# Ego-J/I2VSGG

Measured on AMD Instinct MI355X. Metric: frames/sec (600x1000, 32 ROI/frame), higher is better.
Workload: dtype f32; 1 GPU; BASELINE.json configs[1]: cfgs/res101.yml, SGG_emb fwd+bwd+SGD, 2 frames/GPU 600x1000, 32 boxes + 32 pairs/frame, ResNet-101 C4; frames_per_gpu=2, global_frames=2, hip_graph=True, parallelism=dp1 (frames sharded, RCCL all-reduce of vrd grads)

## Files before the change

### i2vsgg_amd/_lib.py

```python
import ctypes as C
import os

import torch

_HERE = os.path.dirname(os.path.abspath(__file__))
LIB_PATH = os.path.join(_HERE, "libi2vsgg_hip.so")

LAYOUT_NHWC, LAYOUT_NCHW = 0, 1
EPI_RELU, EPI_RESIDUAL, EPI_SCALE, EPI_BIAS, EPI_ZEROED = 1, 2, 4, 8, 16

_p, _i, _f, _z, _l = C.c_void_p, C.c_int32, C.c_float, C.c_size_t, C.c_int64

SIGNATURES = {
    "i2v_version": (_i, []),
    "i2v_last_error": (C.c_char_p, []),
    "i2v_build_flags": (_i, []),
    "i2v_stream_create": (_i, [_i, _i, C.POINTER(C.c_void_p)]),
    "i2v_stream_destroy": (_i, [_p]),
    "i2v_roi_align_fwd": (_i, [_p, _i, _i, _i, _i, _i, _p, _i, _i, _i, _f, _i, _p, _i, _p]),
    "i2v_roi_align_bwd": (_i, [_p, _i, _p, _i, _i, _i, _f, _i, _p, _i, _i, _i, _i, _i, _p]),
    "i2v_roi_align_bwd_gather_workspace_bytes": (_z, [_i, _i, _i, _i, _i]),
    "i2v_roi_align_bwd_gather": (_i, [_p, _p, _i, _i, _i, _f, _i, _p, _i, _i, _i, _i, _p, _z, _p]),
    "i2v_roi_align_sampled_fwd": (_i, [_p, _i, _i, _i, _i, _i, _p, _i, _i, _i, _f, _i, _p, _i, _p]),
    "i2v_roi_align_sampled_bwd": (_i, [_p, _i, _p, _i, _i, _i, _f, _i, _p, _i, _i, _i, _i, _i, _p]),
# ... 20 lines not shown
    "i2v_winograd4_filter": (_i, [_p, _p, _i, _i, _p]),
    "i2v_winograd4_filter_dgrad": (_i, [_p, _p, _i, _i, _p]),
    "i2v_conv3x3_winograd4_workspace_bytes": (_z, [_i, _i, _i, _i, _i]),
    "i2v_conv3x3_winograd4_fwd": (_i, [_p, _p, _p, _p, _p, _i, _i, _i, _i, _i, _i, _p, _z, _p]),
    "i2v_conv_set_tile": (_i, [_i]),
    "i2v_conv_debug_clock": (_i, [_p]),
    "i2v_debug_clock_stamp": (_i, [_p, _p]),
    "i2v_conv_dgrad_workspace_bytes": (_z, [_i, _i, _i, _i]),
    "i2v_conv_dgrad": (_i, [_p, _p, _p, _i, _i, _i, _i, _i, _i, _i, _i, _i, _p, _z, _p, _z, _p]),
    "i2v_conv_wgrad_workspace_bytes": (_z, [_i, _i, _i, _i, _i, _i, _i, _i, _i]),
    "i2v_conv_wgrad": (_i, [_p, _p, _p, _i, _i, _i, _i, _i, _i, _i, _i, _i, _f, _p, _z, _p]),
    "i2v_conv_dgrad_fused": (_i, [_p, _p, _p, _p, _p, _p, _p, _i, _i, _i, _i, _i, _i, _i, _i, _i, _p, _z, _p, _z, _p]),
    "i2v_conv_wgrad_scaled": (_i, [_p, _p, _p, _p, _i, _i, _i, _i, _i, _i, _i, _i, _i, _f, _p, _z, _p]),
    "i2v_ordered_fallbacks": (_i, [_i]),
    "i2v_conv3x3_winograd4_dgrad": (_i, [_p, _p, _p, _p, _p, _i, _i, _i, _i, _i, _p, _z, _p]),
    "i2v_conv3x3_winograd4_wgrad_workspace_bytes": (_z, [_i, _i, _i, _i, _i]),
    "i2v_conv3x3_winograd4_wgrad": (_i, [_p, _p, _p, _p, _i, _i, _i, _i, _i, _f, _p, _z, _p]),
    "i2v_gemm_tn_batched": (_i, [_p, _p, _p, _i, _i, _i, _i, _l, _l, _l, _p]),
    "i2v_gemm_tn_batched_acc": (_i, [_p, _p, _p, _i, _i, _i, _i, _l, _l, _l, _p]),
    "i2v_conv3x3_winograd4_v_bytes": (_z, [_i, _i, _i, _i]),
    "i2v_conv3x3_winograd4_fwd_keep": (_i, [_p, _p, _p, _p, _p, _p, _i, _i, _i, _i, _i, _i, _p, _z, _p]),
    "i2v_conv3x3_winograd4_wgrad_v": (_i, [_p, _p, _p, _p, _i, _i, _i, _i, _i, _f, _p, _z, _p]),
    "i2v_conv_wgrad_sgd": (_i, [_p, _p, _p, _p, _i, _i, _i, _i, _i, _i, _i, _i, _i, _f, _f, _f, _p]),
    "i2v_epilogue_bwd": (_i, [_p, _p, _p, _p, _p, _p, _l, _i, _i, _p, _p, _z, _p]),
    "i2v_maxpool3x3s2_fwd": (_i, [_p, _p, _p, _i, _i, _i, _i, _p]),
    "i2v_sgd_momentum": (_i, [_p, _p, _p, _l, _f, _f, _f, _p]),
    "i2v_sgd_momentum_multi": (_i, [_p, _p, _p, _p, _p, _p, _i, _f, _p]),
    "i2v_adam_step": (_i, [_p, _p]),
    "i2v_adam_multi": (_i, [_p, _p, _p, _p, _p, _p, _p, _i, C.c_double, C.c_double, C.c_double, _p, _p]),
    "i2v_dstyle_pool_fwd": (_i, [_p, _p, _p, _l, _i, _i, _i, _p]),
    "i2v_dstyle_pool_bwd": (_i, [_p, _p, _p, _p, _p, _l, _i, _i, _i, _p]),
    "i2v_dstyle_fused_workspace_bytes": (_z, [_l, _i, _i, _i]),
    "i2v_dstyle_fused_fwd": (_i, [_p, _p, _p, _p, _p, _p, _p, _p, _l, _i, _i, _i, _i, _p, _z, _p]),
    "i2v_relation_topk_workspace_bytes": (_z, [_i, _i]),
    "i2v_relation_topk": (_i, [_p, _p, _p, _p, _i, _i, _i, _p, _p, _p, _p, _z, _p]),
    "i2v_image_prep_size": (_i, [_i, _i, _i, _p, _p, _p]),
    "i2v_image_prep": (_i, [_p, _i, _i, _i, _i, _p, _i, _p, _i, _i, _p]),
    "i2v_det_postprocess_workspace_bytes": (_z, [_i, _i]),
    "i2v_det_postprocess": (_i, [_p, _p, _p, _i, _p, _p, _f, _f, _f, _i, _i, _f, _f, _i, _p, _p, _p, _z, _p]),
    "i2v_det_postprocess_info": (_i, [_p, _p, _p, _i, _p, _p, _p, _i, _i, _f, _f, _i, _p, _p, _p, _z, _p]),
    "i2v_l2norm_rows_fwd": (_i, [_p, _p, _p, _i, _i, _f, _p]),
    "i2v_l2norm_rows_bwd": (_i, [_p, _p, _p, _p, _i, _i, _f, _p]),
    "i2v_bce_rows_fwd": (_i, [_p, _p, _p, _p, _i, _i, _p]),
    "i2v_bce_rows_bwd": (_i, [_p, _p, _p, _p, _p, _i, _i, _p]),
    "i2v_half_mse_fwd": (_i, [_p, _l, _f, _p, _p]),
    "i2v_half_mse_bwd": (_i, [_p, _l, _f, _p, _p, _p]),
    "i2v_smooth_l1_fwd": (_i, [_p, _p, _p, _p, _l, _i, _i, _f, _p, _p]),
    "i2v_smooth_l1_bwd": (_i, [_p, _p, _p, _p, _l, _i, _i, _f, _p, _p, _p]),
    "i2v_bbox_transform": (_i, [_p, _i, _p, _i, _p, _i, _i, _p, _p, _p]),
    "i2v_signed_sqrt_fwd": (_i, [_p, _p, _l, _p]),
    "i2v_signed_sqrt_bwd": (_i, [_p, _p, _p, _l, _p]),
    "i2v_pair_gather_fwd": (_i, [_p, _p, _p, _p, _i, _i, _i, _p]),
    "i2v_pair_gather_bwd": (_i, [_p, _p, _p, _p, _i, _i, _i, _p]),
    "i2v_dpixel_fwd": (_i, [_p, _p, _p, _p, _p, _p, _p, _p, _i, _i, _p]),
    "i2v_dpixel_bwd_workspace_bytes": (_z, []),
    "i2v_dpixel_bwd": (_i, [_p, _p, _p, _p, _p, _p, _p, _p, _p, _p, _p, _p, _i, _i, _f, _p, _z, _p]),
}


class I2VError(RuntimeError):
    pass


def _load():
    if not os.path.exists(LIB_PATH):
        raise ImportError(
            "i2vsgg_amd: %s not found. Build it with `python -c 'import __graft_entry__ as g; g.build()'` "
            "(hipcc --offload-arch=gfx950). There is no CPU fallback." % LIB_PATH)
    lib = C.CDLL(LIB_PATH)
    for name, (res, args) in SIGNATURES.items():
        try:
            fn = getattr(lib, name)
        except AttributeError:
            raise ImportError("i2vsgg_amd: %s does not export %s (stale build?)" % (LIB_PATH, name))
        fn.restype, fn.argtypes = res, args
    return lib


lib = _load()

TUNE = {"I2V_CONV_SPEC": 0, "I2V_SPLIT_TARGET": 1, "I2V_SPLIT_TARGET_SKINNY": 2, "I2V_SPLIT_BELOW": 3, "I2V_SPLIT_ATOMICS": 4,
        "I2V_BIG_FC_TILE": 5, "I2V_WGRAD_V2": 6, "I2V_WGRAD_FUSED_TILE": 7, "I2V_WINO_ROWS": 8, "I2V_ROIPOOL_C128": 9, "I2V_CONV_GEMM": 10, "I2V_STAGGER": 11, "I2V_ROIALIGN_COLS": 12, "I2V_WGRAD_PER_CU": 13, "I2V_WGRAD_XCD": 14, "I2V_FC_FOLD": 15, "I2V_GEMM_X3": 16,
        "I2V_GEMM_PERSIST": 17, "I2V_WGRAD_PRIO": 18, "I2V_STREAM_TILE": 19, "I2V_KGROUPS": 20, "I2V_WGRAD_ORDERED_GFLOP": 21, "I2V_GEMM_DMA": 22,
        "I2V_WGRAD_DMA": 23, "I2V_ROIALIGN_BWD": 24, "I2V_NMS_SCAN": 25}
ENV_TUNE = ("I2V_SPLIT_ATOMICS", "I2V_SPLIT_TARGET", "I2V_SPLIT_TARGET_SKINNY", "I2V_SPLIT_BELOW", "I2V_BIG_FC_TILE",
            "I2V_WGRAD_FUSED_TILE", "I2V_WGRAD_PER_CU", "I2V_KGROUPS", "I2V_WGRAD_ORDERED_GFLOP", "I2V_WINO_ROWS", "I2V_GEMM_DMA", "I2V_WGRAD_DMA", "I2V_ROIALIGN_BWD", "I2V_NMS_SCAN")
RETIRED_ENV = ("I2V_WINOGRAD_TRAIN", "I2V_BLOCK_FUSED", "I2V_WINOGRAD_WGRAD", "I2V_KEEP_V", "I2V_WGRAD_BRANCH", "I2V_ISD_BATCHED",
               "I2V_DEFER_FC", "I2V_EXPERIMENTS")
for _name, _key in TUNE.items():
    if os.environ.get(_name) in (None, ""):
        continue
    if _name not in ENV_TUNE:
        raise ImportError("i2vsgg_amd: %s is set but is not an environment knob (README.md lists them); it would be ignored. "
                          "Use i2vsgg_amd._lib.lib.i2v_set_tuning(TUNE[%r], value) from a tool or test" % (_name, _name))
    if lib.i2v_set_tuning(_key, int(os.environ[_name])) != 0:
        raise ImportError("i2vsgg_amd: %s=%s refused: %s" % (_name, os.environ[_name], lib.i2v_last_error().decode()))
for _name in RETIRED_ENV:
    if os.environ.get(_name) not in (None, ""):
        import warnings
        warnings.warn("i2vsgg_amd: %s is set but no longer read (a settled switch of rounds 1-5): the default runs" % _name)


def check(rc, what):
    if rc != 0:
        raise I2VError("%s failed (%d): %s" % (what, rc, lib.i2v_last_error().decode()))


def ptr(t):
    return None if t is None else t.data_ptr()


def stream():
    import torch
    return torch.cuda.current_stream().cuda_stream
```

### i2vsgg_amd/csrc/api.cpp

```cpp
#include <hip/hip_runtime.h>
#include <stdarg.h>
#include <stdio.h>
#include "../../include/i2vsgg_hip.h"

static thread_local char g_err[512] = "";

void i2v_set_error(const char* fmt, ...) {
    va_list ap;
    va_start(ap, fmt);
    vsnprintf(g_err, sizeof(g_err), fmt, ap);
    va_end(ap);
}

extern "C" int32_t i2v_version(void) { return 100; }
extern "C" const char* i2v_last_error(void) { return g_err; }

int g_i2v_tuning[I2V_TUNE_COUNT] = {
     -1,  2,  -1,  256,  2,
     1,  1,  128,  0,  1,
     1,  0,  2,  4,  1,
     0,  0,  0,  0,  1,
     0,  1000000,  1,  1,  1,  2,
};

extern "C" int32_t i2v_build_flags(void) {
    return 0;
}

extern "C" int32_t i2v_set_tuning(int32_t key, int32_t value) {
    if (key < 0 || key >= I2V_TUNE_COUNT) {
        i2v_set_error("set_tuning: unknown key %d", key);
        return I2V_ERR_ARG;
    }
    const bool retired = key == I2V_TUNE_CONV_SPEC ? value > 0
                       : (key == I2V_TUNE_FC_FOLD || key == I2V_TUNE_GEMM_X3 || key == I2V_TUNE_GEMM_PERSIST ||
                          key == I2V_TUNE_WGRAD_PRIO || key == I2V_TUNE_STAGGER) ? value != 0 : false;
    if (retired) {
        i2v_set_error("set_tuning: key %d belonged to an experiment kernel that is no longer in the library", key);
        return I2V_ERR_UNSUPPORTED;
    }
    g_i2v_tuning[key] = value;
    return I2V_OK;
}


extern "C" int32_t i2v_get_tuning(int32_t key) {
    return (key < 0 || key >= I2V_TUNE_COUNT) ? I2V_ERR_ARG : g_i2v_tuning[key];
}

extern "C" int32_t i2v_stream_create(int32_t device, int32_t priority, void** stream) {
    if (!stream) {
        i2v_set_error("stream_create: null output");
        return I2V_ERR_ARG;
    }
    int prev = -1, n = 0;
    if (hipGetDeviceCount(&n) != hipSuccess || device < 0 || device >= n) {
        i2v_set_error("stream_create: no device %d (%d visible)", device, n);
        return I2V_ERR_ARG;
    }
    hipStream_t s = nullptr;
    hipError_t e = hipGetDevice(&prev);
    if (e == hipSuccess && prev != device) e = hipSetDevice(device);
    if (e == hipSuccess) {
        int lo = 0, hi = 0;
        e = hipDeviceGetStreamPriorityRange(&lo, &hi);
        if (e == hipSuccess) {
            int pr = priority < hi ? hi : (priority > lo ? lo : priority);
            e = hipStreamCreateWithPriority(&s, hipStreamNonBlocking, pr);
        }
    }
    if (prev >= 0 && prev != device) (void)hipSetDevice(prev);
    if (e != hipSuccess) {
        i2v_set_error("stream_create: %s", hipGetErrorString(e));
        return I2V_ERR_LAUNCH;
    }
    *stream = (void*)s;
    return I2V_OK;
}

extern "C" int32_t i2v_stream_destroy(void* stream) {
    if (!stream) return I2V_OK;
    hipError_t e = hipStreamDestroy((hipStream_t)stream);
    if (e != hipSuccess) {
        i2v_set_error("stream_destroy: %s", hipGetErrorString(e));
        return I2V_ERR_LAUNCH;
    }
    return I2V_OK;
}
```

### i2vsgg_amd/csrc/conv.hip

```cpp
#include "common.h"
#include <algorithm>
#include <type_traits>
#include <stdlib.h>

namespace {

typedef float f32x16 __attribute__((ext_vector_type(16)));
typedef float f32x4 __attribute__((ext_vector_type(4)));
typedef unsigned int u32x4 __attribute__((ext_vector_type(4)));
typedef __bf16 bf16x4 __attribute__((ext_vector_type(4)));
typedef __bf16 bf16x8 __attribute__((ext_vector_type(8)));

constexpr int BK = 16;
constexpr int KTAB_MAX = 2560;
constexpr int BKS = 32;
constexpr int LDS_ROW = 20;
constexpr int THREADS = 256;
constexpr int kSplitInKernelMax = 4;

struct ConvP {
    const float* x; const float* w; const float* scale; const float* shift; const float* res; float* y;
    const float* mask;
    int B, H, W, Cin, Cout, KH, KW, stride, pad, Ho, Wo;
    int pad_x;
// ... 1926 lines not shown
            if (gpre) *(float4*)(gpre + r * N + n) = v;
            if (g) *(float4*)(g + r * N + n) = make_float4(v.x * sc.x, v.y * sc.y, v.z * sc.z, v.w * sc.w);
        }
    }
    if (!gbias) return;
    *(float4*)&red[threadIdx.x * 4] = s;
    __syncthreads();
    float4 t = make_float4(0.f, 0.f, 0.f, 0.f);
    if (threadIdx.x < cg) {
        for (int l = 0; l < lanes; ++l) {
            const float4 u = *(const float4*)&red[(l * cg + threadIdx.x) * 4];
            t.x += u.x; t.y += u.y; t.z += u.z; t.w += u.w;
        }
    }
    colsum_finish4(t, (int)(threadIdx.x % cg) * 4, N, threadIdx.x < cg, gbias, part, cnt);
}

__global__ void __launch_bounds__(256)
epilogue_bwd_scalar_kernel(const float* __restrict__ gy, const float* __restrict__ y, const float* __restrict__ scale,
                           float* __restrict__ g, float* __restrict__ gpre, float* __restrict__ gbias, long long M,
                           int N, int relu, int rows_per_blk, float* __restrict__ g_t, float* __restrict__ part) {
    const int n = blockIdx.y * 256 + threadIdx.x;
    if (n >= N) return;
    const long long r0 = (long long)blockIdx.x * rows_per_blk;
    const long long r1 = r0 + rows_per_blk < M ? r0 + rows_per_blk : M;
    const float sc = scale ? scale[n] : 1.f;
    float s = 0.f;
    for (long long r = r0; r < r1; ++r) {
        float v = gy[r * N + n];
        if (relu && !(y[r * N + n] > 0.f)) v = 0.f;
        s += v;
        if (gpre) gpre[r * N + n] = v;
        if (g) g[r * N + n] = v * sc;
        if (g_t) g_t[(long long)n * M + r] = v * sc;
    }
    if (gbias && part) part[(long long)blockIdx.x * N + n] = s;
    else if (gbias) atomicAdd(gbias + n, s);
}

}


extern "C" int32_t i2v_ordered_fallbacks(int32_t reset) {
    const int n = g_ordered_fallbacks;
    if (reset) g_ordered_fallbacks = 0;
    return n;
}

namespace {
__global__ void __launch_bounds__(256)
wgrad_reduce_kernel(const float* __restrict__ part, float* __restrict__ gw, int splits, int planes, long long nk4, long long bsw, int acc) {
    const long long total = (long long)planes * nk4;
    for (long long e = blockIdx.x * 256ll + threadIdx.x; e < total; e += 256ll * gridDim.x) {
        const long long plane = e / nk4, i = e - plane * nk4;
        float4* o = (float4*)(gw + plane * bsw) + i;
        float4 v = acc ? *o : make_float4(0.f, 0.f, 0.f, 0.f);
        const float4* src = (const float4*)part + plane * nk4 + i;
        for (int s0 = 0; s0 < splits; s0 += 8) {
            float4 u[8];
#pragma unroll
            for (int k = 0; k < 8; ++k) u[k] = s0 + k < splits ? src[(long long)(s0 + k) * planes * nk4] : make_float4(0.f, 0.f, 0.f, 0.f);
#pragma unroll
            for (int k = 0; k < 8; ++k)
                if (s0 + k < splits) { v.x += u[k].x; v.y += u[k].y; v.z += u[k].z; v.w += u[k].w; }
        }
        *o = v;
    }
}
__global__ void __launch_bounds__(256)
wgrad_reduce_scalar_kernel(const float* __restrict__ part, float* __restrict__ gw, int splits, long long nk, int acc) {
    for (long long e = blockIdx.x * 256ll + threadIdx.x; e < nk; e += 256ll * gridDim.x) {
        float v = acc ? gw[e] : 0.f;
        for (int s0 = 0; s0 < splits; s0 += 16) {
            float u[16];
#pragma unroll
            for (int k = 0; k < 16; ++k) u[k] = s0 + k < splits ? part[(long long)(s0 + k) * nk + e] : 0.f;
#pragma unroll
            for (int k = 0; k < 16; ++k)
                if (s0 + k < splits) v += u[k];
        }
        gw[e] = v;
    }
}
}

constexpr int kWgradOrderedMax = 16;

static int wgrad_split_count(long long M, int N, int K, int planes, int tm, int tk, int rs) {
    const long long tiles = (long long)i2v_cdiv(N, tm) * i2v_cdiv(K, tk), all_tiles = tiles * planes;
    const int msteps = i2v_cdiv(M, rs), per_cu = g_i2v_tuning[I2V_TUNE_WGRAD_PER_CU];
    int splits = (int)((long long)per_cu * NUM_CU / all_tiles);
    if (splits < 2) splits = (int)(((long long)per_cu * NUM_CU + all_tiles - 1) / all_tiles);
    if (splits > msteps / 4) splits = msteps / 4;
    if (splits < 1) splits = 1;
    return splits;
}

int i2v_internal_wgrad_plane_splits(long long T, int Cout, int Cin) {
    const int s = wgrad_split_count(T, Cout, Cin, 36, 64, 64, BKS);
    const int mps = i2v_cdiv(i2v_cdiv(T, BKS), s) * BKS;
    return i2v_cdiv(T, mps);
}

static bool launch_wgrad(WgP& p, float beta, bool fused, hipStream_t st, void* split_ws = nullptr, size_t split_ws_bytes = 0) {
    const long long xb = (long long)p.B * p.H * p.W * p.Cin * 4, gb = (long long)p.M * p.N * 4;
    const bool v2 = (p.N % 4 == 0) && xb < (1ll << 31) && gb < (1ll << 31) && g_wgrad_v2;
    if (p.row_scale && !v2) { i2v_set_error("conv_wgrad_scaled: shape outside the v2 kernel (Cout % 4, 2 GiB operands)"); return false; }
    int tm = 64, tk = 64;
    if (v2 && fused && g_wgrad_fused_tile == 128 && p.N >= 128) tm = 128;
    if (v2 && g_wgrad_v2 >= 2) {
        if (p.N >= 128) tm = 128;
        if (p.K >= 128 && tm == 128 && g_wgrad_v2 == 2) tk = 128;
    }
    const long long tiles = (long long)i2v_cdiv(p.N, tm) * i2v_cdiv(p.K, tk);
    const int rs = v2 ? BKS : 16;
    int splits = 1;
    const int msteps = i2v_cdiv(p.M, rs);
    if (!fused) splits = wgrad_split_count(p.M, p.N, p.K, p.nbatch > 1 ? p.nbatch : 1, tm, tk, rs);
    const int planes = p.nbatch > 1 ? p.nbatch : 1;
    const bool ext_part = p.part_ws != nullptr;
    const double ord_flops = 1e9 * g_i2v_tuning[I2V_TUNE_WGRAD_ORDERED_GFLOP], flops = 2.0 * p.M * p.N * p.K * planes;
    const bool want_ord = !fused && !ext_part && splits > 1 && g_i2v_tuning[I2V_TUNE_SPLIT_ATOMICS] == 0 && flops < ord_flops;
    if (want_ord && split_ws && v2 && splits > kWgradOrderedMax && flops < 1e9) splits = kWgradOrderedMax;
    if (ext_part && splits > p.part_cap) splits = p.part_cap > 0 ? p.part_cap : 1;
    p.m_per_split = i2v_cdiv(msteps, splits) * rs;
    splits = i2v_cdiv(p.M, p.m_per_split);
    p.direct = (splits == 1 && beta == 0.f) || fused;
    bool two_pass = false;
    if (ext_part) {
        if (splits == 1) p.part_ws = nullptr;
    } else if (want_ord && splits > 1) {
        const size_t need_ord = kSplitCounterBytes + (size_t)splits * tiles * planes * (size_t)(tm * tk) * sizeof(float);
        const size_t need_part = kSplitCounterBytes + (size_t)splits * planes * (size_t)p.N * p.K * sizeof(float);
        if (split_ws && v2 && splits <= kWgradOrderedMax && tiles * planes <= kSplitCounters && need_ord <= split_ws_bytes && need_ord < (1ull << 31)) {
            p.ord_cnt = reinterpret_cast<int*>(split_ws);
            p.ord_ws = reinterpret_cast<float*>(static_cast<char*>(split_ws) + kSplitCounterBytes);
            p.ord_splits = splits; p.ord_tiles = (int)tiles; p.ord_acc = beta != 0.f;
        } else if (split_ws && need_part <= split_ws_bytes) {
            p.part_ws = reinterpret_cast<float*>(static_cast<char*>(split_ws) + kSplitCounterBytes);
            two_pass = true;
        } else {
            ++g_ordered_fallbacks;
        }
    }
    if (beta == 0.f && !p.direct && !p.ord_ws && !p.part_ws)
        hipMemsetAsync(p.gw, 0, (p.nbatch > 1 ? (size_t)(p.nbatch - 1) * p.bsw : 0) * sizeof(float) + (size_t)p.N * p.K * sizeof(float), st);
    p.x_bytes = (unsigned)xb;
    p.gy_bytes = (unsigned)gb;
    dim3 grid((unsigned)tiles, splits, p.nbatch > 1 ? p.nbatch : 1);
    const long long groups = (long long)splits * (p.nbatch > 1 ? p.nbatch : 1), total = tiles * groups;
    p.xcd_remap = (v2 && groups >= 2 && total < (1ll << 30) && g_i2v_tuning[I2V_TUNE_WGRAD_XCD]) ? 1 : 0;
    if (p.xcd_remap) {
        p.r_tiles = (int)tiles; p.r_splits = splits; p.r_total = (int)total;
        grid = dim3((unsigned)((total + 7) / 8 * 8), 1, 1);
    }
    const bool lin = p.KH == 1 && p.KW == 1 && p.pad == 0 && p.stride == 1;
    const bool dma = v2 && !fused && !g_clk && lin && (p.K % 4 == 0) && g_i2v_tuning[I2V_TUNE_WGRAD_DMA];
    if (!v2) conv_wgrad_f32<64, 64><<<grid, THREADS, 0, st>>>(p);
    else if (dma && tm == 128 && tk == 128) conv_wgrad2_f32<4, 4, false, false, true><<<grid, THREADS, 0, st>>>(p);
    else if (dma && tm == 128) conv_wgrad2_f32<4, 2, false, false, true><<<grid, THREADS, 0, st>>>(p);
    else if (dma) conv_wgrad2_f32<2, 2, false, false, true><<<grid, THREADS, 0, st>>>(p);
    else if (fused && tm == 128 && tk == 64) conv_wgrad2_f32<4, 2, true><<<grid, THREADS, 0, st>>>(p);
    else if (tm == 128 && tk == 128) conv_wgrad2_f32<4, 4><<<grid, THREADS, 0, st>>>(p);
    else if (tm == 128) conv_wgrad2_f32<4, 2><<<grid, THREADS, 0, st>>>(p);
    else if (fused) conv_wgrad2_f32<2, 2, true><<<grid, THREADS, 0, st>>>(p);
    else if (g_clk) { p.clk = g_clk; p.abl = g_ablate; conv_wgrad2_f32<2, 2, false, true><<<grid, THREADS, 0, st>>>(p); }
// ... 239 lines not shown
    return I2V_OK;
}

static int32_t gemm_tn_batched_impl(const float* x, const float* gy, float* gw, int32_t M, int32_t N, int32_t K, int32_t nbatch,
                                    long long stride_x, long long stride_gy, long long stride_gw, float beta, void* stream,
                                    int part_cap = 0, int* part_splits = nullptr) {
    I2V_CHECK_ARG(x && gy && gw && M > 0 && N > 0 && K > 0 && nbatch > 0, "gemm_tn_batched: bad argument");
    I2V_CHECK_ARG(N % 4 == 0 && K % 4 == 0, "gemm_tn_batched: N and K must be multiples of 4");
    I2V_CHECK_ARG(nbatch == 1 || stride_gw == (long long)N * K, "gemm_tn_batched: gw batches must be contiguous");
    WgP p = {};
    p.x = x; p.gy = gy; p.gw = gw;
    p.B = 1; p.H = 1; p.W = M; p.Cin = K; p.Cout = N; p.KH = 1; p.KW = 1; p.stride = 1; p.pad = 0;
    p.Ho = 1; p.Wo = M;
    p.M = M; p.N = N; p.K = K;
    p.lgCin = ilog2_exact(K);
    p.nbatch = nbatch; p.bsx = stride_x; p.bsg = stride_gy; p.bsw = stride_gw;
    if (!g_wgrad_v2 || (long long)M * K * 4 >= (1ll << 31) || (long long)M * N * 4 >= (1ll << 31)) {
        i2v_set_error("gemm_tn_batched: operand larger than 2 GiB per batch");
        return I2V_ERR_UNSUPPORTED;
    }
    if (part_splits) {
        p.part_ws = gw; p.part_cap = part_cap;
    }
    launch_wgrad(p, beta, false, (hipStream_t)stream);
    if (part_splits) *part_splits = p.part_ws ? p.ord_splits : 1;
    I2V_CHECK_LAUNCH("gemm_tn_batched");
    return I2V_OK;
}

int32_t i2v_internal_reduce_parts(float* parts, int nparts, int planes, long long nk, void* stream) {
    const long long total = (long long)planes * (nk / 4);
    wgrad_reduce_kernel<<<(unsigned)std::min<long long>(i2v_cdiv(total, 256), 4096), 256, 0, (hipStream_t)stream>>>(
        parts, parts, nparts, planes, nk / 4, nk, 0);
    return I2V_OK;
}

int32_t i2v_internal_gemm_tn_batched_parts(const float* x, const float* gy, float* parts, int32_t M, int32_t N, int32_t K,
                                           int32_t nbatch, long long stride_x, long long stride_gy, int cap, int* splits, void* stream) {
    return gemm_tn_batched_impl(x, gy, parts, M, N, K, nbatch, stride_x, stride_gy, (long long)N * K, 0.f, stream, cap, splits);
}

extern "C" int32_t i2v_gemm_tn_batched(const float* x, const float* gy, float* gw, int32_t M, int32_t N, int32_t K,
                                       int32_t nbatch, long long stride_x, long long stride_gy, long long stride_gw,
                                       void* stream) {
    return gemm_tn_batched_impl(x, gy, gw, M, N, K, nbatch, stride_x, stride_gy, stride_gw, 0.f, stream);
}

extern "C" int32_t i2v_gemm_tn_batched_acc(const float* x, const float* gy, float* gw, int32_t M, int32_t N, int32_t K,
                                           int32_t nbatch, long long stride_x, long long stride_gy, long long stride_gw,
                                           void* stream) {
    return gemm_tn_batched_impl(x, gy, gw, M, N, K, nbatch, stride_x, stride_gy, stride_gw, 1.f, stream);
}

extern "C" int32_t i2v_conv_wgrad(const float* x, const float* gy, float* gw, int32_t B, int32_t H, int32_t W,
                                  int32_t Cin, int32_t Cout, int32_t KH, int32_t KW, int32_t stride, int32_t pad,
                                  float beta, void* ws, size_t ws_bytes, void* stream) {
    return conv_wgrad_impl(x, gy, gw, nullptr, B, H, W, Cin, Cout, KH, KW, stride, pad, beta, stream, ws, ws_bytes);
}

extern "C" int32_t i2v_conv_wgrad_scaled(const float* x, const float* gy, const float* row_scale, float* gw, int32_t B,
                                         int32_t H, int32_t W, int32_t Cin, int32_t Cout, int32_t KH, int32_t KW,
                                         int32_t stride, int32_t pad, float beta, void* ws, size_t ws_bytes, void* stream) {
    return conv_wgrad_impl(x, gy, gw, row_scale, B, H, W, Cin, Cout, KH, KW, stride, pad, beta, stream, ws, ws_bytes);
}

extern "C" int32_t i2v_conv_wgrad_sgd(const float* x, const float* gy, float* w, float* m, int32_t B, int32_t H,
                                      int32_t W, int32_t Cin, int32_t Cout, int32_t KH, int32_t KW, int32_t stride,
                                      int32_t pad, float lr, float momentum, float weight_decay, void* stream) {
    int rc = check_conv("conv_wgrad_sgd", x, gy, w, B, H, W, Cin, Cout, KH, KW, stride, pad);
    if (rc) return rc;
    I2V_CHECK_ARG(m, "conv_wgrad_sgd: null momentum buffer");
    WgP p = {};
    p.x = x; p.gy = gy; p.gw = w; p.sgd_m = m; p.lr = lr; p.mom = momentum; p.wd = weight_decay;
    p.B = B; p.H = H; p.W = W; p.Cin = Cin; p.Cout = Cout; p.KH = KH; p.KW = KW; p.stride = stride; p.pad = pad;
    p.Ho = (H + 2 * pad - KH) / stride + 1;
    p.Wo = (W + 2 * pad - KW) / stride + 1;
    p.M = B * p.Ho * p.Wo; p.N = Cout; p.K = KH * KW * Cin;
    p.lgCin = ilog2_exact(Cin);
    const long long tiles = (long long)i2v_cdiv(p.N, 64) * i2v_cdiv(p.K, 64);
    if (tiles < 2 * NUM_CU || p.M > 4096) {
        i2v_set_error("conv_wgrad_sgd: shape needs a split over pixels; use i2v_conv_wgrad + i2v_sgd_momentum");
        return I2V_ERR_UNSUPPORTED;
    }
    launch_wgrad(p, 0.f, true, (hipStream_t)stream);
    I2V_CHECK_LAUNCH("conv_wgrad_sgd");
    return I2V_OK;
}

extern "C" int32_t i2v_epilogue_bwd(const float* gy, const float* y, const float* scale, float* g, float* gpre,
                                    float* gbias, int64_t M, int32_t N, int32_t relu, float* g_t, void* split_ws,
                                    size_t split_ws_bytes, void* stream) {
    I2V_CHECK_ARG(gy && M >= 0 && N > 0, "epilogue_bwd: bad argument");
    I2V_CHECK_ARG(!relu || y, "epilogue_bwd: relu needs y");
    if (M == 0) return I2V_OK;
    const bool vec = (N & 3) == 0;
    const int cols = vec ? 1024 : 256;
    const bool want_ord = gbias && vec && g_i2v_tuning[I2V_TUNE_SPLIT_ATOMICS] == 0;
    const bool small = M * (long long)N <= (1ll << 21);
    auto ordered = [&](long long nblk, int ncolblk, float*& part, int*& cnt) {
        part = nullptr; cnt = nullptr;
        if (!want_ord || nblk < 2) return;
        const long long groups = (nblk + kColsumGroup - 1) / kColsumGroup;
        const size_t need = kSplitCounterBytes + (size_t)(nblk + groups) * N * sizeof(float);
        if (!split_ws || (long long)ncolblk * (1 + groups) > kSplitCounters || need > split_ws_bytes || need >= (1ull << 31)) {
            ++g_ordered_fallbacks;
            return;
        }
        cnt = reinterpret_cast<int*>(split_ws);
        part = reinterpret_cast<float*>(static_cast<char*>(split_ws) + kSplitCounterBytes);
    };
    float* part; int* cnt;
    int rows = 64;
    while (rows > 4 && (long long)i2v_cdiv(M, rows) * i2v_cdiv(N, cols) < 2 * NUM_CU) rows >>= 1;
    if (vec && N <= 512 && M >= 1024 && !g_t) {
        const int lanes = 256 / (N >> 2);
        int rpb = lanes * 64;
        while (rpb > lanes && i2v_cdiv(M, rpb) < 48) rpb >>= 1;
        if (want_ord && small) while (i2v_cdiv(M, rpb) > 64) rpb <<= 1;
        ordered(i2v_cdiv(M, rpb), 1, part, cnt);
        epilogue_bwd_narrow_kernel<<<(unsigned)i2v_cdiv(M, rpb), 256, 0, (hipStream_t)stream>>>(gy, y, scale, g, gpre,
                                                                                              gbias, M, N, relu, rpb, part, cnt);
        I2V_CHECK_LAUNCH("epilogue_bwd");
        return I2V_OK;
    }
    if (want_ord && vec && small) while (i2v_cdiv(M, rows) > 32 && rows < 1024) rows <<= 1;
    dim3 grid(i2v_cdiv(M, rows), i2v_cdiv(N, cols));
    ordered(grid.x, (int)grid.y, part, cnt);
    if (vec) {
        epilogue_bwd_kernel<<<grid, 256, 0, (hipStream_t)stream>>>(gy, y, scale, g, gpre, gbias, M, N, relu, rows, g_t, part, cnt);
    } else {
        float* sp = nullptr;
        if (gbias && grid.x > 1 && g_i2v_tuning[I2V_TUNE_SPLIT_ATOMICS] == 0) {
            if (split_ws && kSplitCounterBytes + (size_t)grid.x * N * sizeof(float) <= split_ws_bytes)
                sp = reinterpret_cast<float*>(static_cast<char*>(split_ws) + kSplitCounterBytes);
            else ++g_ordered_fallbacks;
        }
        epilogue_bwd_scalar_kernel<<<grid, 256, 0, (hipStream_t)stream>>>(gy, y, scale, g, gpre, gbias, M, N, relu, rows, g_t, sp);
        if (sp) wgrad_reduce_scalar_kernel<<<(unsigned)i2v_cdiv(N, 256), 256, 0, (hipStream_t)stream>>>(sp, gbias, (int)grid.x, N, 1);
    }
    I2V_CHECK_LAUNCH("epilogue_bwd");
    return I2V_OK;
}

extern "C" int32_t i2v_maxpool3x3s2_fwd(const float* x, float* y, int32_t* argmax, int32_t B, int32_t H, int32_t W,
                                        int32_t C, void* stream) {
    I2V_CHECK_ARG(x && y && B > 0 && H >= 3 && W >= 3 && C > 0 && C % 4 == 0, "maxpool: bad argument");
    int Ho = (H - 3 + 1) / 2 + 1, Wo = (W - 3 + 1) / 2 + 1;
    if ((Ho - 1) * 2 >= H) --Ho;
    if ((Wo - 1) * 2 >= W) --Wo;
    const long long total = (long long)B * Ho * Wo * (C / 4);
    maxpool3x3s2_kernel<<<(int)fmin((double)i2v_cdiv(total, 256), 8192.0), 256, 0, (hipStream_t)stream>>>(
        x, y, argmax, B, H, W, C, Ho, Wo);
    I2V_CHECK_LAUNCH("maxpool3x3s2");
    return I2V_OK;
}

extern "C" int32_t i2v_sgd_momentum_multi(float* const* p, const float* const* g, float* const* m, const int64_t* n,
                                          const float* lr, const float* weight_decay, int32_t count, float momentum,
                                          void* stream) {
    I2V_CHECK_ARG(count >= 0 && (count == 0 || (p && g && m && n && lr && weight_decay)), "sgd_momentum_multi: bad argument");
    for (int32_t c0 = 0; c0 < count; c0 += SGD_MULTI_MAX) {
        SgdMulti t;
        t.count = 0;
        t.mom = momentum;
        int blocks = 0;
        for (int32_t c = c0; c < count && t.count < SGD_MULTI_MAX; ++c) {
            I2V_CHECK_ARG(p[c] && g[c] && m[c] && n[c] >= 0, "sgd_momentum_multi: bad tensor");
// ... 63 lines not shown
```

### include/i2vsgg_hip.h

```cpp
#ifndef I2VSGG_HIP_H
#define I2VSGG_HIP_H

#include <stdint.h>
#include <stddef.h>

#ifdef __cplusplus
extern "C" {
#endif

#define I2V_OK               0
#define I2V_ERR_ARG         -1
#define I2V_ERR_LAUNCH      -2
#define I2V_ERR_WORKSPACE   -3
#define I2V_ERR_UNSUPPORTED -4

#define I2V_LAYOUT_NHWC 0
#define I2V_LAYOUT_NCHW 1

#define I2V_EPI_RELU      1
#define I2V_EPI_RESIDUAL  2
#define I2V_EPI_SCALE     4
#define I2V_EPI_BIAS      8
#define I2V_EPI_ZEROED   16
#define I2V_EPI_MASK     32
// ... 35 lines not shown
                              float* out, int32_t* argmax, int32_t out_layout, void* stream);
int32_t i2v_roi_pool_bwd(const float* grad_out, const int32_t* argmax, int32_t out_layout,
                         const float* rois, int32_t R, int32_t pooled_h, int32_t pooled_w,
                         float* grad_feat, int32_t feat_layout, int32_t B, int32_t C, int32_t H, int32_t W,
                         void* stream);

size_t  i2v_nms_workspace_bytes(int32_t n_img, int32_t n);
int32_t i2v_nms_sorted(const float* dets, int32_t n_img, int32_t n, float thresh, int32_t max_keep,
                       int32_t* keep_out, int32_t* num_out, void* workspace, size_t workspace_bytes,
                       void* stream);

size_t  i2v_rpn_proposal_workspace_bytes(int32_t B, int32_t H, int32_t W, int32_t A, int32_t pre_nms_top_n);
int32_t i2v_rpn_proposal(const float* cls, int32_t is_prob, const float* bbox, const float* im_info,
                         const float* base_anchors, int32_t B, int32_t H, int32_t W, int32_t A,
                         int32_t feat_stride, int32_t pre_nms_top_n, int32_t post_nms_top_n, float nms_thresh,
                         float* rois, int32_t* kept_idx, int32_t* num_kept,
                         void* workspace, size_t workspace_bytes, void* stream);

int32_t i2v_rpn_decode(const float* cls, int32_t is_prob, const float* bbox, const float* im_info,
                       const float* base_anchors, int32_t B, int32_t H, int32_t W, int32_t A, int32_t feat_stride,
                       float* proposals , float* scores , void* stream);
size_t  i2v_sort_desc_workspace_bytes(int32_t n_seg, int32_t n);
int32_t i2v_sort_desc(const float* keys, int32_t n_seg, int32_t n, int32_t* order_out ,
                      void* workspace, size_t workspace_bytes, void* stream);

int32_t i2v_image_prep_size(int32_t H, int32_t W, int32_t target_size, int32_t* Ho, int32_t* Wo, float* scale);
int32_t i2v_image_prep(const uint8_t* img, int32_t H, int32_t W, int32_t rgb_order, int32_t flipped,
                       const float* pixel_means_bgr, int32_t target_size, float* blob, int32_t blob_h,
                       int32_t blob_w, void* stream);

size_t  i2v_det_postprocess_workspace_bytes(int32_t R, int32_t C);
int32_t i2v_det_postprocess(const float* rois, const float* cls_prob, const float* bbox_pred, int32_t class_agnostic,
                            const float* stds, const float* means, float im_h, float im_w, float im_scale,
                            int32_t R, int32_t C, float score_thresh, float nms_thresh, int32_t max_per_image,
                            float* dets, int32_t* counts, void* workspace, size_t workspace_bytes, void* stream);
int32_t i2v_det_postprocess_info(const float* rois, const float* cls_prob, const float* bbox_pred, int32_t class_agnostic,
                                 const float* stds, const float* means, const float* im_info,
                                 int32_t R, int32_t C, float score_thresh, float nms_thresh, int32_t max_per_image,
                                 float* dets, int32_t* counts, void* workspace, size_t workspace_bytes, void* stream);

size_t  i2v_relation_topk_workspace_bytes(int32_t n_pairs, int32_t n_rel);
int32_t i2v_relation_topk(const float* rel_score, const float* conf, const int64_t* ixs, const int64_t* ixo,
                          int32_t n_pairs, int32_t n_rel, int32_t k, int32_t* pair_out, int32_t* pred_out,
                          float* conf_out, void* workspace, size_t workspace_bytes, void* stream);

int32_t i2v_bbox_overlaps(const float* boxes, int32_t box_stride, int32_t box_off, int32_t boxes_batched,
                          const float* gt, int32_t B, int32_t N, int32_t K,
                          float* overlaps, float* max_ov, int32_t* argmax_ov, void* stream);

int32_t i2v_conv_fwd(const float* x, const float* w, const float* scale, const float* shift, const float* res,
                     float* y, int32_t B, int32_t H, int32_t W, int32_t Cin, int32_t Cout,
                     int32_t KH, int32_t KW, int32_t stride, int32_t pad, int32_t flags,
                     void* split_workspace, size_t split_workspace_bytes, void* stream);
int32_t i2v_conv_fwd_splits(int32_t B, int32_t H, int32_t W, int32_t Cin, int32_t Cout, int32_t KH, int32_t KW,
                            int32_t stride, int32_t pad, size_t ws_bytes);
size_t  i2v_conv_split_workspace_bytes(int32_t B, int32_t H, int32_t W, int32_t Cin, int32_t Cout, int32_t KH,
                                       int32_t KW, int32_t stride, int32_t pad);
#define I2V_TUNE_CONV_SPEC            0
#define I2V_TUNE_SPLIT_TARGET         1
#define I2V_TUNE_SPLIT_TARGET_SKINNY  2
#define I2V_TUNE_SPLIT_BELOW          3
#define I2V_TUNE_SPLIT_ATOMICS        4
#define I2V_TUNE_BIG_FC_TILE          5
#define I2V_TUNE_WGRAD_V2             6
#define I2V_TUNE_WGRAD_FUSED_TILE     7
#define I2V_TUNE_WINO_ROWS            8
#define I2V_TUNE_ROIPOOL_C128         9
#define I2V_TUNE_CONV_GEMM           10
#define I2V_TUNE_STAGGER             11
#define I2V_TUNE_ROIALIGN_COLS       12
#define I2V_TUNE_WGRAD_PER_CU        13
#define I2V_TUNE_WGRAD_XCD           14
#define I2V_TUNE_FC_FOLD             15
#define I2V_TUNE_GEMM_X3             16
#define I2V_TUNE_GEMM_PERSIST        17
#define I2V_TUNE_WGRAD_PRIO          18
#define I2V_TUNE_STREAM_TILE         19
#define I2V_TUNE_KGROUPS             20
#define I2V_TUNE_WGRAD_ORDERED_GFLOP 21
#define I2V_TUNE_GEMM_DMA            22
#define I2V_TUNE_WGRAD_DMA           23
#define I2V_TUNE_ROIALIGN_BWD        24
#define I2V_TUNE_NMS_SCAN            25
#define I2V_TUNE_COUNT               26
int32_t i2v_set_tuning(int32_t key, int32_t value);
int32_t i2v_get_tuning(int32_t key);
int32_t i2v_conv_set_tile(int32_t cfg);
int32_t i2v_conv_debug_clock(void* buf);
int32_t i2v_debug_clock_stamp(void* out2, void* stream);
int32_t i2v_conv_dgrad_fused(const float* gy, const float* w, const float* gy_scale, const float* out_scale,
                             const float* res, const float* mask, float* gx, int32_t B, int32_t H, int32_t W,
                             int32_t Cin, int32_t Cout, int32_t KH, int32_t KW, int32_t stride, int32_t pad,
                             void* workspace, size_t workspace_bytes, void* split_workspace, size_t split_workspace_bytes,
                             void* stream);
int32_t i2v_conv_wgrad_scaled(const float* x, const float* gy, const float* row_scale, float* gw, int32_t B,
                              int32_t H, int32_t W, int32_t Cin, int32_t Cout, int32_t KH, int32_t KW,
                              int32_t stride, int32_t pad, float beta, void* split_workspace, size_t split_workspace_bytes,
                              void* stream);
int32_t i2v_ordered_fallbacks(int32_t reset);
int32_t i2v_conv3x3_winograd4_dgrad(const float* gy, const float* U, const float* out_scale, const float* mask,
                                    float* gx, int32_t B, int32_t H, int32_t W, int32_t Cout, int32_t Cin,
                                    void* workspace, size_t workspace_bytes, void* stream);
size_t  i2v_conv3x3_winograd4_wgrad_workspace_bytes(int32_t B, int32_t H, int32_t W, int32_t Cin, int32_t Cout);
int32_t i2v_conv3x3_winograd4_wgrad(const float* x, const float* gy, const float* row_scale, float* gw,
                                    int32_t B, int32_t H, int32_t W, int32_t Cin, int32_t Cout, float beta,
                                    void* workspace, size_t workspace_bytes, void* stream);
size_t  i2v_conv3x3_winograd4_v_bytes(int32_t B, int32_t H, int32_t W, int32_t Cin);
int32_t i2v_conv3x3_winograd4_fwd_keep(const float* x, const float* U, const float* scale, const float* shift,
                                       float* y, float* v_out, int32_t B, int32_t H, int32_t W, int32_t Cin,
                                       int32_t Cout, int32_t relu, void* workspace, size_t workspace_bytes, void* stream);
int32_t i2v_conv3x3_winograd4_wgrad_v(const float* v, const float* gy, const float* row_scale, float* gw,
                                      int32_t B, int32_t H, int32_t W, int32_t Cin, int32_t Cout, float beta,
                                      void* workspace, size_t workspace_bytes, void* stream);
int32_t i2v_gemm_tn_batched(const float* x, const float* gy, float* gw, int32_t M, int32_t N, int32_t K,
                            int32_t nbatch, long long stride_x, long long stride_gy, long long stride_gw, void* stream);
int32_t i2v_gemm_tn_batched_acc(const float* x, const float* gy, float* gw, int32_t M, int32_t N, int32_t K,
                            int32_t nbatch, long long stride_x, long long stride_gy, long long stride_gw, void* stream);
size_t  i2v_conv_dgrad_workspace_bytes(int32_t Cin, int32_t Cout, int32_t KH, int32_t KW);
int32_t i2v_conv_dgrad(const float* gy, const float* w, float* gx, int32_t B, int32_t H, int32_t W,
                       int32_t Cin, int32_t Cout, int32_t KH, int32_t KW, int32_t stride, int32_t pad,
                       void* workspace, size_t workspace_bytes, void* split_workspace, size_t split_workspace_bytes,
                       void* stream);
size_t  i2v_conv_wgrad_workspace_bytes(int32_t B, int32_t H, int32_t W, int32_t Cin, int32_t Cout,
                                       int32_t KH, int32_t KW, int32_t stride, int32_t pad);
int32_t i2v_conv_wgrad(const float* x, const float* gy, float* gw, int32_t B, int32_t H, int32_t W,
                       int32_t Cin, int32_t Cout, int32_t KH, int32_t KW, int32_t stride, int32_t pad,
                       float beta, void* workspace, size_t workspace_bytes, void* stream);

int32_t i2v_gemm_nt_batched(const float* a, const float* b, float* c, int32_t M, int32_t N, int32_t K, int32_t nbatch,
                            int64_t stride_a, int64_t stride_b, int64_t stride_c,
                            void* split_workspace, size_t split_workspace_bytes, void* stream);

int32_t i2v_winograd_filter(const float* w, float* U, int32_t Cout, int32_t Cin, void* stream);
size_t  i2v_conv3x3_winograd_workspace_bytes(int32_t B, int32_t H, int32_t W, int32_t Cin, int32_t Cout);
int32_t i2v_conv3x3_winograd_fwd(const float* x, const float* U, const float* scale, const float* shift, float* y,
                                 int32_t B, int32_t H, int32_t W, int32_t Cin, int32_t Cout, int32_t relu,
                                 void* workspace, size_t workspace_bytes, void* stream);

int32_t i2v_winograd4_filter(const float* w, float* U, int32_t Cout, int32_t Cin, void* stream);
int32_t i2v_winograd4_filter_dgrad(const float* w, float* U, int32_t Cout, int32_t Cin, void* stream);
size_t  i2v_conv3x3_winograd4_workspace_bytes(int32_t B, int32_t H, int32_t W, int32_t Cin, int32_t Cout);
int32_t i2v_conv3x3_winograd4_fwd(const float* x, const float* U, const float* scale, const float* shift, float* y,
                                  int32_t B, int32_t H, int32_t W, int32_t Cin, int32_t Cout, int32_t relu,
                                  void* workspace, size_t workspace_bytes, void* stream);

int32_t i2v_conv_wgrad_sgd(const float* x, const float* gy, float* w, float* m, int32_t B, int32_t H, int32_t W,
                           int32_t Cin, int32_t Cout, int32_t KH, int32_t KW, int32_t stride, int32_t pad,
                           float lr, float momentum, float weight_decay, void* stream);

int32_t i2v_epilogue_bwd(const float* gy, const float* y, const float* scale, float* g, float* gpre, float* gbias,
                         int64_t M, int32_t N, int32_t relu, float* g_t, void* split_ws, size_t split_ws_bytes, void* stream);

int32_t i2v_maxpool3x3s2_fwd(const float* x, float* y, int32_t* argmax, int32_t B, int32_t H, int32_t W, int32_t C,
                             void* stream);

int32_t i2v_dstyle_pool_fwd(const float* x1, const float* x2, float* z, int64_t rows, int32_t n_img,
                            int32_t dim, int32_t rank, void* stream);
int32_t i2v_dstyle_pool_bwd(const float* gz, const float* x1, const float* x2, float* g1, float* g2,
                            int64_t rows, int32_t n_img, int32_t dim, int32_t rank, void* stream);
size_t  i2v_dstyle_fused_workspace_bytes(int64_t rows, int32_t n_img, int32_t dim, int32_t rank);
int32_t i2v_dstyle_fused_fwd(const float* x, const float* w1, const float* b1, const float* w2, const float* b2,
                             float* z, float* x1, float* x2, int64_t rows, int32_t n_img, int32_t k, int32_t dim,
                             int32_t rank, void* workspace, size_t workspace_bytes, void* stream);

int32_t i2v_l2norm_rows_fwd(const float* x, float* y, float* inv_norm, int32_t rows, int32_t cols, float eps, void* stream);
int32_t i2v_l2norm_rows_bwd(const float* g, const float* y, const float* inv_norm, float* gx, int32_t rows, int32_t cols,
                            float eps, void* stream);
// ... 45 lines not shown
```

Before: 485.9 frames/s.

## Add fused FC weight-gradient plus SGD momentum update kernel for small-M linear layers

Adds a dedicated MFMA kernel for 1x1 linear layers with at most 256 rows. It computes the weight gradient tile in registers and applies the momentum SGD update directly, streaming weights and momentum with non-temporal buffer loads and stores. Work is split into strips over N and chunks over K, with XCD-aware block grouping and double-buffered LDS for x. It replaces the generic wgrad+SGD path when the new tuning key is on (default on), targeting the bandwidth-bound FC update; the fallback remains for other shapes.

```diff
diff --git a/i2vsgg_amd/_lib.py b/i2vsgg_amd/_lib.py
--- a/i2vsgg_amd/_lib.py
+++ b/i2vsgg_amd/_lib.py
@@ -126,7 +126,7 @@
 TUNE = {"I2V_CONV_SPEC": 0, "I2V_SPLIT_TARGET": 1, "I2V_SPLIT_TARGET_SKINNY": 2, "I2V_SPLIT_BELOW": 3, "I2V_SPLIT_ATOMICS": 4,
         "I2V_BIG_FC_TILE": 5, "I2V_WGRAD_V2": 6, "I2V_WGRAD_FUSED_TILE": 7, "I2V_WINO_ROWS": 8, "I2V_ROIPOOL_C128": 9, "I2V_CONV_GEMM": 10, "I2V_STAGGER": 11, "I2V_ROIALIGN_COLS": 12, "I2V_WGRAD_PER_CU": 13, "I2V_WGRAD_XCD": 14, "I2V_FC_FOLD": 15, "I2V_GEMM_X3": 16,
         "I2V_GEMM_PERSIST": 17, "I2V_WGRAD_PRIO": 18, "I2V_STREAM_TILE": 19, "I2V_KGROUPS": 20, "I2V_WGRAD_ORDERED_GFLOP": 21, "I2V_GEMM_DMA": 22,
-        "I2V_WGRAD_DMA": 23, "I2V_ROIALIGN_BWD": 24, "I2V_NMS_SCAN": 25}
+        "I2V_WGRAD_DMA": 23, "I2V_ROIALIGN_BWD": 24, "I2V_NMS_SCAN": 25, "I2V_FC_UPDATE": 26}
 ENV_TUNE = ("I2V_SPLIT_ATOMICS", "I2V_SPLIT_TARGET", "I2V_SPLIT_TARGET_SKINNY", "I2V_SPLIT_BELOW", "I2V_BIG_FC_TILE",
             "I2V_WGRAD_FUSED_TILE", "I2V_WGRAD_PER_CU", "I2V_KGROUPS", "I2V_WGRAD_ORDERED_GFLOP", "I2V_WINO_ROWS", "I2V_GEMM_DMA", "I2V_WGRAD_DMA", "I2V_ROIALIGN_BWD", "I2V_NMS_SCAN")
 RETIRED_ENV = ("I2V_WINOGRAD_TRAIN", "I2V_BLOCK_FUSED", "I2V_WINOGRAD_WGRAD", "I2V_KEEP_V", "I2V_WGRAD_BRANCH", "I2V_ISD_BATCHED",
diff --git a/i2vsgg_amd/csrc/api.cpp b/i2vsgg_amd/csrc/api.cpp
--- a/i2vsgg_amd/csrc/api.cpp
+++ b/i2vsgg_amd/csrc/api.cpp
@@ -21,6 +21,7 @@
      1,  0,  2,  4,  1,
      0,  0,  0,  0,  1,
      0,  1000000,  1,  1,  1,  2,
+     1,
 };
 
 extern "C" int32_t i2v_build_flags(void) {
diff --git a/i2vsgg_amd/csrc/conv.hip b/i2vsgg_amd/csrc/conv.hip
--- a/i2vsgg_amd/csrc/conv.hip
+++ b/i2vsgg_amd/csrc/conv.hip
@@ -2032,6 +2032,160 @@
         gw[e] = v;
     }
 }
+constexpr int FCU_WAVES = 8, FCU_THREADS = 64 * FCU_WAVES, FCU_BN = 16 * FCU_WAVES, FCU_TK = 64;
+struct FcuP {
+    const float* x; const float* gy; float* w; float* m;
+    float lr, mom, wd;
+    int M, N, K;
+    int strips, chunks, tiles, groups;
+    unsigned x_bytes, gy_bytes, w_bytes;
+};
+
+template <int NS>
+__global__ void __launch_bounds__(FCU_THREADS) fc_update_f32(const FcuP p) {
+    const int L = (int)blockIdx.x, g = L & 7, r = L >> 3;
+    const int start = (int)(((long long)g * p.groups) >> 3), count = (int)(((long long)(g + 1) * p.groups) >> 3) - start;
+    if (r >= count) return;
+    const int idx = start + r, chunk = idx / p.strips, strip = idx - chunk * p.strips;
+    const int t0 = (int)((long long)chunk * p.tiles / p.chunks), t1 = (int)((long long)(chunk + 1) * p.tiles / p.chunks);
+
+    constexpr unsigned MASK = 0x80000000u, NT = 2;
+    constexpr int ROWS = 32 * NS;
+    __shared__ __attribute__((aligned(16))) float xs[2][ROWS * FCU_TK];
+    const int tid = threadIdx.x, lane = tid & 63, wave = tid >> 6, fr = lane & 15, fg = lane >> 4;
+    const int n0 = strip * FCU_BN;
+    const __amdgpu_buffer_rsrc_t gr = __builtin_amdgcn_make_buffer_rsrc((void*)p.gy, 0, p.gy_bytes, 0x00020000);
+    const __amdgpu_buffer_rsrc_t xr = __builtin_amdgcn_make_buffer_rsrc((void*)p.x, 0, p.x_bytes, 0x00020000);
+    const __amdgpu_buffer_rsrc_t wr = __builtin_amdgcn_make_buffer_rsrc((void*)p.w, 0, p.w_bytes, 0x00020000);
+    const __amdgpu_buffer_rsrc_t mr = __builtin_amdgcn_make_buffer_rsrc((void*)p.m, 0, p.w_bytes, 0x00020000);
+
+    float a[NS * 8];
+    {
+        const unsigned na = (unsigned)(n0 + 16 * wave + fr);
+        const bool nin = (int)na < p.N;
+#pragma unroll
+        for (int st = 0; st < NS; ++st)
+#pragma unroll
+            for (int q = 0; q < 8; ++q) {
+                const unsigned row = (unsigned)(32 * st + 16 * (q >> 2) + 4 * fg + (q & 3));
+                const unsigned off = ((row * (unsigned)p.N + na) * 4u) | ((nin && (int)row < p.M) ? 0u : MASK);
+                a[st * 8 + q] = __builtin_bit_cast(float, __builtin_amdgcn_raw_buffer_load_b32(gr, off, 0, 0));
+            }
+    }
+
+    float4 xv[NS];
+    auto xload = [&](int t) {
+        const unsigned k = (unsigned)(t * FCU_TK + 4 * (tid & 15));
+        const bool kin = t < t1 && (int)k < p.K;
+#pragma unroll
+        for (int q = 0; q < NS; ++q) {
+            const unsigned row = (unsigned)((tid >> 4) + 32 * q);
+            const unsigned off = ((row * (unsigned)p.K + k) * 4u) | ((kin && (int)row < p.M) ? 0u : MASK);
+            xv[q] = __builtin_bit_cast(float4, __builtin_amdgcn_raw_buffer_load_b128(xr, off, 0, 0));
+        }
+    };
+    auto xstore = [&](int buf) {
+#pragma unroll
+        for (int q = 0; q < NS; ++q) *(float4*)&xs[buf][((tid >> 4) + 32 * q) * FCU_TK + 4 * (tid & 15)] = xv[q];
+    };
+    auto wm_offsets = [&](int t, unsigned (&off)[4]) {
+        const unsigned k = (unsigned)(t * FCU_TK + 4 * fr);
+        const bool kin = t < t1 && (int)k < p.K;
+#pragma unroll
+        for (int q = 0; q < 4; ++q) {
+            const unsigned n = (unsigned)(n0 + 16 * wave + 4 * fg + q);
+            off[q] = ((n * (unsigned)p.K + k) * 4u) | ((kin && (int)n < p.N) ? 0u : MASK);
+        }
+    };
+    auto wm_load = [&](int t, float4 (&wv)[4], float4 (&mv)[4]) {
+        unsigned off[4];
+        wm_offsets(t, off);
+#pragma unroll
+        for (int q = 0; q < 4; ++q) {
+            wv[q] = __builtin_bit_cast(float4, __builtin_amdgcn_raw_buffer_load_b128(wr, off[q], 0, NT));
+            mv[q] = __builtin_bit_cast(float4, __builtin_amdgcn_raw_buffer_load_b128(mr, off[q], 0, NT));
+        }
+    };
+
+    int buf = 0;
+    auto body = [&](int t, float4 (&wv)[4], float4 (&mv)[4]) {
+        f32x4 acc[4];
+#pragma unroll
+        for (int j = 0; j < 4; ++j) acc[j] = (f32x4){0.f, 0.f, 0.f, 0.f};
+#pragma unroll
+        for (int st = 0; st < NS; ++st) {
+            float4 b[8];
+#pragma unroll
+            for (int q = 0; q < 8; ++q) b[q] = *(const float4*)&xs[buf][(32 * st + 16 * (q >> 2) + 4 * fg + (q & 3)) * FCU_TK + 4 * fr];
+#pragma unroll
+            for (int q = 0; q < 8; ++q) {
+                acc[0] = __builtin_amdgcn_mfma_f32_16x16x4f32(a[st * 8 + q], b[q].x, acc[0], 0, 0, 0);
+                acc[1] = __builtin_amdgcn_mfma_f32_16x16x4f32(a[st * 8 + q], b[q].y, acc[1], 0, 0, 0);
+                acc[2] = __builtin_amdgcn_mfma_f32_16x16x4f32(a[st * 8 + q], b[q].z, acc[2], 0, 0, 0);
+                acc[3] = __builtin_amdgcn_mfma_f32_16x16x4f32(a[st * 8 + q], b[q].w, acc[3], 0, 0, 0);
+            }
+        }
+        __builtin_amdgcn_sched_barrier(0);
+        unsigned off[4];
+        wm_offsets(t, off);
+#pragma unroll
+        for (int q = 0; q < 4; ++q) {
+            float4 pv = wv[q], m4 = mv[q];
+            m4.x = p.mom * m4.x + (acc[0][q] + p.wd * pv.x); m4.y = p.mom * m4.y + (acc[1][q] + p.wd * pv.y);
+            m4.z = p.mom * m4.z + (acc[2][q] + p.wd * pv.z); m4.w = p.mom * m4.w + (acc[3][q] + p.wd * pv.w);
+            pv.x -= p.lr * m4.x; pv.y -= p.lr * m4.y; pv.z -= p.lr * m4.z; pv.w -= p.lr * m4.w;
+            __builtin_amdgcn_raw_buffer_store_b128(__builtin_bit_cast(u32x4, m4), mr, off[q], 0, NT);
+            __builtin_amdgcn_raw_buffer_store_b128(__builtin_bit_cast(u32x4, pv), wr, off[q], 0, NT);
+        }
+        xstore(buf ^ 1);
+        xload(t + 2);
+        wm_load(t + 2, wv, mv);
+        __syncthreads();
+        buf ^= 1;
+    };
+
+    float4 wA[4], mA[4], wB[4], mB[4];
+    xload(t0);
+    __builtin_amdgcn_s_waitcnt(0);
+    xstore(0);
+    xload(t0 + 1);
+    wm_load(t0, wA, mA);
+    wm_load(t0 + 1, wB, mB);
+    __syncthreads();
+    for (int t = t0;; t += 2) {
+        body(t, wA, mA);
+        if (t + 1 >= t1) break;
+        body(t + 1, wB, mB);
+        if (t + 2 >= t1) break;
+    }
+}
+}
+
+static bool launch_fc_update(const WgP& p, hipStream_t st) {
+    if (!g_i2v_tuning[I2V_TUNE_FC_UPDATE] || !g_wgrad_v2) return false;
+    const bool lin = p.KH == 1 && p.KW == 1 && p.pad == 0 && p.stride == 1;
+    const long long xb = (long long)p.M * p.K * 4, gb = (long long)p.M * p.N * 4, wb = (long long)p.N * p.K * 4;
+    if (!lin || p.M > 256 || p.N % 4 || p.K % 4 || xb >= (1ll << 31) || gb >= (1ll << 31) || wb >= (1ll << 31)) return false;
+    FcuP q = {};
+    q.x = p.x; q.gy = p.gy; q.w = p.gw; q.m = p.sgd_m; q.lr = p.lr; q.mom = p.mom; q.wd = p.wd;
+    q.M = p.M; q.N = p.N; q.K = p.K;
+    q.strips = i2v_cdiv(p.N, FCU_BN);
+    q.tiles = i2v_cdiv(p.K, FCU_TK);
+    q.chunks = std::min(std::max(NUM_CU / q.strips, 1), q.tiles);
+    q.groups = q.strips * q.chunks;
+    q.x_bytes = (unsigned)xb; q.gy_bytes = (unsigned)gb; q.w_bytes = (unsigned)wb;
+    const unsigned grid = (unsigned)((q.groups + 7) / 8 * 8);
+    switch (i2v_cdiv(p.M, 32)) {
+    case 1: fc_update_f32<1><<<grid, FCU_THREADS, 0, st>>>(q); break;
+    case 2: fc_update_f32<2><<<grid, FCU_THREADS, 0, st>>>(q); break;
+    case 3: fc_update_f32<3><<<grid, FCU_THREADS, 0, st>>>(q); break;
+    case 4: fc_update_f32<4><<<grid, FCU_THREADS, 0, st>>>(q); break;
+    case 5: fc_update_f32<5><<<grid, FCU_THREADS, 0, st>>>(q); break;
+    case 6: fc_update_f32<6><<<grid, FCU_THREADS, 0, st>>>(q); break;
+    case 7: fc_update_f32<7><<<grid, FCU_THREADS, 0, st>>>(q); break;
+    default: fc_update_f32<8><<<grid, FCU_THREADS, 0, st>>>(q); break;
+    }
+    return true;
 }
 
 constexpr int kWgradOrderedMax = 16;
@@ -2437,7 +2591,7 @@
         i2v_set_error("conv_wgrad_sgd: shape needs a split over pixels; use i2v_conv_wgrad + i2v_sgd_momentum");
         return I2V_ERR_UNSUPPORTED;
     }
-    launch_wgrad(p, 0.f, true, (hipStream_t)stream);
+    if (!launch_fc_update(p, (hipStream_t)stream)) launch_wgrad(p, 0.f, true, (hipStream_t)stream);
     I2V_CHECK_LAUNCH("conv_wgrad_sgd");
     return I2V_OK;
 }
diff --git a/include/i2vsgg_hip.h b/include/i2vsgg_hip.h
--- a/include/i2vsgg_hip.h
+++ b/include/i2vsgg_hip.h
@@ -141,7 +141,8 @@
 #define I2V_TUNE_WGRAD_DMA           23
 #define I2V_TUNE_ROIALIGN_BWD        24
 #define I2V_TUNE_NMS_SCAN            25
-#define I2V_TUNE_COUNT               26
+#define I2V_TUNE_FC_UPDATE           26
+#define I2V_TUNE_COUNT               27
 int32_t i2v_set_tuning(int32_t key, int32_t value);
 int32_t i2v_get_tuning(int32_t key);
 int32_t i2v_conv_set_tile(int32_t cfg);
```

New measurement: 509.9 frames/s, median of 6. 4.9% higher.
